# bhavyageethika/multimodal_autonomous_driving_perception_and_planning

Measured on AMD Instinct MI355X. Metric: end-to-end frames/sec (1280x720 synthetic), higher is better.
Workload: dtype f64; 1 GPU; config4: 64 stream(s)/GPU x 1-frame window per step, 1280x720, simulated detection + IoU tracker + 6-state KF + 21-candidate planner, one launch per step, up to 4 consecutive steps in flight; streams_per_gpu=64, window=1, graph=False, taggers=False, allgather_track_tables=False, fused_step=True, overlapped_steps=4, steps_per_library_call=8, parallelism=stream-sharded x1

## Files before the change

### include/avhot.h

```cpp
#ifndef AVHOT_H
#define AVHOT_H

#include <stddef.h>
#include <stdint.h>

#ifdef __cplusplus
extern "C" {
#endif

#define AV_VERSION 102

enum {
    AV_OK = 0,
    AV_EINVAL = -1,
    AV_EHIP = -2,
    AV_ENODEV = -3,
    AV_ESTATE = -4,
    AV_ENOMEM = -5
};

typedef struct av_ctx av_ctx;
typedef void* av_stream_t;

int av_version(void);
// ... 320 lines not shown
    int32_t type;
    int32_t x0, y0, x1, y1, x2, y2, x3, y3;
    int32_t p;
    uint8_t b, g, r, a;
    int32_t reserved;
} av_prim;
int av_raster_draw(av_ctx* ctx, av_stream_t stream, int n_images, int h, int w, uint8_t* img, const av_prim* prims, int prim_cap,
                   const int32_t* n_prims, const int32_t* verts, int vert_cap);
typedef struct {
    int32_t width, height;
    double pixels_per_meter;
    double x_min, x_max, y_min, y_max;
    int32_t n_candidates;
    int32_t reserved;
} av_bev_cfg;
int av_bev_prim_cap(const av_bev_cfg* cfg, int tcap, int n_points);
int av_bev_build(av_ctx* ctx, av_stream_t stream, const av_bev_cfg* cfg, int n_streams, int n_frames, int frame, int tcap,
                 int trajectory_length, const av_track_row* snap, const int32_t* snap_n, const void* tracker_state,
                 const double* vstate, const double* waypoints, const int32_t* order, av_prim* prims, int prim_cap, int32_t* n_prims);
int av_resize_into(av_ctx* ctx, av_stream_t stream, const uint8_t* src, int sh, int sw, uint8_t* dst, int dh, int dw, int dst_pitch_px,
                   int dst_x0);

int av_i420_to_bgr(av_ctx* ctx, av_stream_t stream, int n_frames, int h, int w, const uint8_t* yuv, uint8_t* bgr);

int av_synth_frames(av_ctx* ctx, av_stream_t stream, int n_streams, int h, int w, int stream0, int frame,
                    uint8_t* bgr);

int av_hot_step(av_ctx* ctx, av_stream_t stream, const av_tracker_cfg* tracker_cfg, const av_kf_cfg* kf_cfg, int n_streams, int h,
                int w, int dcap, int tcap, int32_t* frame_count, int32_t* det_n, int32_t* det_box, int32_t* det_cls,
                double* det_conf, int32_t* det_status, void* tracker_state, av_track_row* snap, int32_t* snap_n, int32_t* det2trk,
                const double* z, double* kf_state, double* vstate, double* plan_state, double* waypoints, double* cost,
                int32_t* order, void* wire, int stream0, int frame0);
int av_hot_step_fits(av_ctx* ctx, int n_streams, int dcap, int tcap, int depth);

#define AV_STEP_FLAG_INTS(n_streams) (65 * (n_streams) + 32 + 64)
int av_hot_step_seq(av_ctx* ctx, av_stream_t stream, const av_tracker_cfg* tracker_cfg, const av_kf_cfg* kf_cfg, int n_streams, int h,
                    int w, int dcap, int tcap, int32_t* frame_count, int32_t* det_n, int32_t* det_box, int32_t* det_cls,
                    double* det_conf, int32_t* det_status, void* tracker_state, av_track_row* snap, int32_t* snap_n, int32_t* det2trk,
                    const double* z, double* kf_state, double* vstate, double* plan_state, double* waypoints, double* cost,
                    int32_t* order, void* wire, int stream0, int frame0, int32_t* seq_flags, int seq, int depth);

#define AV_STEP_MAX_DEPTH 4
typedef struct av_step_set {
    int32_t *det_n, *det_box, *det_cls;
    double* det_conf;
    av_track_row* snap;
    int32_t *snap_n, *det2trk;
    const double* z;
    double *vstate, *plan_state, *waypoints, *cost;
    int32_t* order;
} av_step_set;
int av_hot_steps_seq(av_ctx* ctx, int depth, const av_stream_t* streams, const av_tracker_cfg* tracker_cfg, const av_kf_cfg* kf_cfg,
                     int n_streams, int h, int w, int dcap, int tcap, int32_t* frame_count, int32_t* det_status, void* tracker_state,
                     double* kf_state, const av_step_set* sets, const double* z_steps, void* wire_steps, int stream0, int frame0,
                     int32_t* seq_flags, int seq0, int n_steps);

#ifdef __cplusplus
}
#endif
#endif
```

### multimodal_autonomous_driving_perception_and_planning_amd/_native.py

```python
import ctypes as C
import os

_HERE = os.path.dirname(os.path.abspath(__file__))
LIB_PATH = os.path.join(_HERE, "libavhot.so")

c_i32p = C.POINTER(C.c_int32)
c_f64p = C.POINTER(C.c_double)
vp = C.c_void_p


class TrackerCfg(C.Structure):
    _fields_ = [("iou_threshold", C.c_double), ("max_age", C.c_int32), ("min_hits", C.c_int32),
                ("trajectory_length", C.c_int32)]


class KfCfg(C.Structure):
    _fields_ = [("dt", C.c_double), ("process_noise", C.c_double), ("measurement_noise", C.c_double)]


class PlannerCfg(C.Structure):
    _fields_ = [("planning_horizon", C.c_double), ("dt", C.c_double), ("num_samples", C.c_int32),
                ("reserved", C.c_int32), ("w_lateral", C.c_double), ("w_velocity", C.c_double),
                ("w_acceleration", C.c_double), ("w_curvature", C.c_double)]

# ... 84 lines not shown
    ("av_stream_sync", C.c_int, [vp]),
    ("av_stream_sync_spin", C.c_int, [vp]),
    ("av_host_alloc", C.c_int, [C.POINTER(vp), C.c_size_t]),
    ("av_host_free", C.c_int, [vp]),
    ("av_copy_h2d", C.c_int, [vp, vp, C.c_size_t, vp]),
    ("av_copy_d2h", C.c_int, [vp, vp, C.c_size_t, vp, C.c_int]),
    ("av_simdet_generate", C.c_int, [vp, vp, C.c_int, C.c_int, C.c_int, C.c_int, C.c_int, vp, vp, vp, vp, vp, vp]),
    ("av_tracker_state_bytes", C.c_size_t, [C.c_int, C.c_int]),
    ("av_tracker_reset", C.c_int, [vp, vp, C.c_int, C.c_int, C.c_int, vp]),
    ("av_tracker_update", C.c_int, [vp, vp, C.POINTER(TrackerCfg), C.c_int, C.c_int, C.c_int, vp, vp, vp, vp,
                                    C.c_int, vp, vp, vp, vp]),
    ("av_wire_table_bytes", C.c_size_t, [C.c_int]),
    ("av_pack_tracks", C.c_int, [vp, vp, C.c_int, C.c_int, C.c_int, C.c_int, C.c_int, C.c_int, C.c_int, vp, vp, vp, vp]),
    ("av_comm_unique_id", C.c_int, [vp]),
    ("av_comm_create", C.c_int, [vp, vp, C.c_int, C.c_int, C.POINTER(vp)]),
    ("av_comm_destroy", C.c_int, [vp]),
    ("av_allgather_tracks", C.c_int, [vp, vp, vp, vp, vp, C.c_size_t]),
    ("av_kf_reset", C.c_int, [vp, vp, C.c_int, vp]),
    ("av_kf_step", C.c_int, [vp, vp, C.POINTER(KfCfg), C.c_int, C.c_int, vp, vp, vp, vp, vp]),
    ("av_planner_configure", C.c_int, [vp, C.POINTER(PlannerCfg)]),
    ("av_planner_dims", C.c_int, [vp, C.POINTER(C.c_int), C.POINTER(C.c_int)]),
    ("av_planner_launch_shape", C.c_int, [C.c_int, C.c_int, C.c_int, C.c_int, c_i32p]),
    ("av_planner_plan", C.c_int, [vp, vp, C.c_int, vp, vp, C.c_int, vp, C.c_int, vp, vp, vp]),
    ("av_planner_plan_each", C.c_int, [vp, vp, C.c_int, vp, vp, vp, C.c_int, C.c_int, vp, vp, C.c_int, vp, vp, vp]),
    ("av_track_obstacles", C.c_int, [vp, vp, C.POINTER(ObstacleCfg), C.c_int, C.c_int, vp, vp, vp, C.c_int, vp, vp]),
    ("av_planner_plan_moving", C.c_int, [vp, vp, C.c_int, vp, vp, vp, C.c_int, C.c_int, vp, vp, C.c_int, vp, vp, vp]),
    ("av_track_obstacles_moving", C.c_int, [vp, vp, C.POINTER(ObstacleCfg), C.c_double, C.c_int, C.c_int, vp, vp, vp, C.c_int, vp,
                                            vp]),
    ("av_dets_to_tracker", C.c_int, [vp, vp, C.c_int, C.c_int, vp, vp, vp, vp, vp, C.c_int, C.c_int, vp, vp, vp, vp, vp]),
    ("av_lane_paths", C.c_int, [vp, vp, C.POINTER(ObstacleCfg), C.c_int, C.c_int, C.c_int, C.c_int, vp, vp, vp, vp, C.c_int,
                                C.c_int, vp, vp, vp]),
    ("av_hot_step", C.c_int, [vp, vp, C.POINTER(TrackerCfg), C.POINTER(KfCfg)] + [C.c_int] * 5 + [vp] * 17 + [vp, C.c_int, C.c_int]),
    ("av_hot_step_fits", C.c_int, [vp, C.c_int, C.c_int, C.c_int, C.c_int]),
    ("av_hot_steps_seq", C.c_int, [vp, C.c_int, vp, C.POINTER(TrackerCfg), C.POINTER(KfCfg)] + [C.c_int] * 5 + [vp] * 7 +
     [C.c_int, C.c_int, vp, C.c_int, C.c_int]),
    ("av_hot_step_seq", C.c_int, [vp, vp, C.POINTER(TrackerCfg), C.POINTER(KfCfg)] + [C.c_int] * 5 + [vp] * 17 +
     [vp, C.c_int, C.c_int, vp, C.c_int, C.c_int]),
    ("av_planner_generate", C.c_int, [vp, vp, C.c_int, vp, vp, vp, vp]),
    ("av_planner_evaluate", C.c_int, [vp, vp, C.c_int, C.c_int, vp, vp, C.c_int, vp, C.c_int, vp]),
    ("av_planner_evaluate_moving", C.c_int, [vp, vp, C.c_int, C.c_int, vp, vp, C.c_int, vp, C.c_int, vp]),
    ("av_lane_workspace_bytes", C.c_size_t, [C.c_int, C.c_int, C.c_int, C.c_int]),
    ("av_lane_workspace_init", C.c_int, [vp, vp, C.c_int, C.c_int, C.c_int, C.c_int, vp]),
    ("av_lane_workspace_view", C.c_int, [C.c_int, C.c_int, C.c_int, C.c_int, C.c_int, C.POINTER(C.c_size_t),
                                         C.POINTER(C.c_size_t)]),
    ("av_raster_draw", C.c_int, [vp, vp, C.c_int, C.c_int, C.c_int, vp, vp, C.c_int, vp, vp, C.c_int]),
    ("av_bev_prim_cap", C.c_int, [vp, C.c_int, C.c_int]),
    ("av_bev_build", C.c_int, [vp, vp, vp, C.c_int, C.c_int, C.c_int, C.c_int, C.c_int, vp, vp, vp, vp, vp, vp, vp, C.c_int, vp]),
    ("av_i420_to_bgr", C.c_int, [vp, vp, C.c_int, C.c_int, C.c_int, vp, vp]),
    ("av_resize_into", C.c_int, [vp, vp, vp, C.c_int, C.c_int, vp, C.c_int, C.c_int, C.c_int, C.c_int]),
    ("av_synth_frames", C.c_int, [vp, vp, C.c_int, C.c_int, C.c_int, C.c_int, C.c_int, vp]),
    ("av_maneuver_reset", C.c_int, [vp, vp, C.c_int, vp]),
    ("av_interaction_state_bytes", C.c_size_t, [C.c_int]),
    ("av_interaction_reset", C.c_int, [vp, vp, C.c_int, C.c_int, vp]),
    ("av_interaction_detect", C.c_int, [vp, vp, vp, C.c_int, C.c_int, C.c_int, vp, vp, vp, vp, vp, vp, vp, vp]),
    ("av_maneuver_detect", C.c_int, [vp, vp, C.c_int, C.c_int, vp, vp, vp, vp]),
    ("av_yolo_param_count", C.c_size_t, []),
    ("av_yolo_create", C.c_int, [vp, C.c_int, C.c_int, C.c_int, vp, C.c_size_t, C.POINTER(vp)]),
    ("av_yolo_create_ex", C.c_int, [vp, C.c_int, C.c_int, C.c_int, vp, C.c_size_t, C.c_int, C.POINTER(vp)]),
    ("av_yolo_destroy", C.c_int, [vp]),
    ("av_yolo_dims", C.c_int, [vp, C.POINTER(C.c_int), C.POINTER(C.c_int), C.POINTER(C.c_int)]),
    ("av_yolo_forward", C.c_int, [vp, vp, vp, C.c_float, C.c_float, C.c_int, vp, vp, vp, vp]),
    ("av_yolo_keep_logits", C.c_int, [vp, C.c_int]),
    ("av_yolo_defer_tail", C.c_int, [vp, C.c_int]),
    ("av_yolo_join_tail", C.c_int, [vp, vp]),
    ("av_yolo_tensor", C.c_int, [vp, C.c_int, C.POINTER(vp)] + [C.POINTER(C.c_int)] * 5),
    ("av_lane_detect", C.c_int, [vp, vp, C.POINTER(LaneCfg), C.c_int, C.c_int, C.c_int, vp, vp, vp, vp, vp, vp, vp,
# ... 41 lines not shown
    except OSError:
        pass


def lib():
    global _lib
    if _lib is not None:
        return _lib
    if not os.path.exists(LIB_PATH):
        raise ImportError(
            "libavhot.so is missing (%s). Build it with `python -c 'import __graft_entry__ as g; g.build()'` "
            "-- this package has no CPU fallback." % LIB_PATH)
    _preload_hip_runtime()
    L = C.CDLL(LIB_PATH)
    for name, res, args in _SIGS + _OPTIONAL_SIGS:
        fn = getattr(L, name)
        fn.restype = res
        fn.argtypes = args
    _lib = L
    return L


def register(sigs):
    global _lib
    _OPTIONAL_SIGS.extend(sigs)
    if _lib is not None:
        for name, res, args in sigs:
            fn = getattr(_lib, name)
            fn.restype = res
            fn.argtypes = args


def step_flag_ints(n_streams):
    return 65 * n_streams + 32 + 64


def step_i32(v):
    v &= 0xFFFFFFFF
    return v - (1 << 32) if v & 0x80000000 else v


class StepSet(C.Structure):
    _fields_ = [(k, C.c_void_p) for k in ("det_n", "det_box", "det_cls", "det_conf", "snap", "snap_n", "det2trk", "z", "vstate",
                                          "plan_state", "waypoints", "cost", "order")]


def check(rc):
    if rc != 0:
        raise RuntimeError("libavhot: %s (code %d)" % (lib().av_last_error_string().decode(), rc))


def ptr(t):
    if t is None:
        return None
    return C.c_void_p(t.data_ptr())


class Context:

    def __init__(self, device=0):
        L = lib()
        h = vp()
        check(L.av_ctx_create(int(device), C.byref(h)))
        self.handle = h
        self.device = int(device)
        s = vp()
        check(L.av_side_stream(h, C.byref(s)))
# ... 32 lines not shown
```

### multimodal_autonomous_driving_perception_and_planning_amd/csrc/planner.hip

```cpp
#include "common.h"

#include <cmath>



namespace {

struct PlanParams {
    int n, n_lat, C;
    double dt, H;
    double w_lat, w_vel, w_acc, w_curv;
    const double *t, *alpha, *q, *dtd, *lat;
    double atq[20];
};

static const double ATAN_Q[20] = {
    -0x1.5555555555549p-2, 0x1.99999999979b9p-3,  -0x1.24924923e22b4p-3, 0x1.c71c718e5a102p-4,
    -0x1.745d120df88fbp-4, 0x1.3b1362fc35ab5p-4,  -0x1.110deef367776p-4, 0x1.e1b3c8d50e91fp-5,
    -0x1.ae2c7119eb922p-5, 0x1.81fdd2525246ap-5,  -0x1.56daf4786fd80p-5, 0x1.2575526b2309ap-5,
    -0x1.d168e01adf666p-6, 0x1.462cc26bda000p-6,  -0x1.8055065b73333p-7, 0x1.693bd6b79999ap-8,
    -0x1.fdf4e15cccccdp-10, 0x1.f224118000000p-12, -0x1.2568700000000p-14, 0x1.2ed799999999ap-18,
};

__device__ __forceinline__ double atan2_fast(double y, double x, const double (&Q)[20]) {
// ... 125 lines not shown
        f = __builtin_amdgcn_readfirstlane(f);
        PlanLists l{nullptr, 0, nullptr, 0};
        if (ref) {
            const int pth = f / ref_stride;
            l.n_ref = path_points(pth);
            l.ref = ref + (size_t)pth * rcap * 2;
        }
        if (obs) {
            const int k = n_obs[f];
            l.n_obs = k < 0 ? 0 : (k > ocap ? ocap : k);
            l.obs = obs + (size_t)f * ocap * OS;
        }
        return l;
    }
};
using PlanEach = PlanEachT<3>;
using PlanEachMoving = PlanEachT<5>;

template <int G, int NW, class Hook = PlanNoHook, class Lists = PlanShared>
__device__ __forceinline__ void plan_block_lists(const PlanParams& p, int f0, int n_states, const double* __restrict__ state,
                                                 const Lists lists, double* __restrict__ wp, double* __restrict__ cost,
                                                 int32_t* __restrict__ order, double* sm, int state_f0 = -1, int rot = 0,
                                                 Hook after1 = Hook()) {
    const int n = p.n, C = p.C;
    const int sd = state_f0 < 0 ? 0 : state_f0 - f0;
    double* vs = sm;
    double* base = vs + (size_t)G * 3 * n * 2;
    double* trig = base + even_up(G * 3 * 3);
    double* costs = trig + G * 8;
    double* stage_all = costs + 3 * even_up(G * C);
    const int CS = even_up(G * C);

    const int tid = threadIdx.x, lane = tid & 63;
    double* stage = stage_all + (size_t)(tid >> 6) * n * 6;
    const int wid = ((tid >> 6) + NW - rot) % NW;
    constexpr int P = G * 3;
    static_assert(NW >= 2, "the heading terms take the last wave");

    auto bcast = [&](double x, int i) {
        const unsigned lo = (unsigned)__builtin_amdgcn_readlane((int)(unsigned)__double_as_longlong(x), i);
        const unsigned hi = (unsigned)__builtin_amdgcn_readlane((int)(unsigned)((unsigned long long)__double_as_longlong(x) >> 32), i);
        return __longlong_as_double((long long)(((unsigned long long)hi << 32) | lo));
    };
    auto terms = [&](double v0, double dv, int i, double& v, double& vdt, double& velt, double& acct) {
        v = blend_velocity(v0, dv, p.alpha[i]);
        vdt = v * p.dt;
        velt = velocity_term(p.w_vel, v);
        acct = 0.0;
        if (i > 0)
            acct = acceleration_term(p.w_acc, v, blend_velocity(v0, dv, p.alpha[i - 1]), p.dtd[i]);
    };
    auto cost_chains = [&](double velt, double acct, unsigned long long hasm, double* b) {
        double sv = 0.0;
#pragma unroll
        for (int i = 0; i < 64; ++i)
            if (i < n) sv = sv + bcast(velt, i);
        double run = sv, sa = 0.0;
#pragma unroll
        for (int i = 1; i < 64; ++i)
            if (i < n && ((hasm >> i) & 1ull)) {
                const double term = bcast(acct, i);
                run = run + term, sa = sa + term;
            }
        if (lane == 0) b[0] = sv, b[1] = sa, b[2] = run;
    };

    const bool fast = n <= 64 && P <= NW;
    double k_velt = 0.0, k_acct = 0.0;
    unsigned long long k_has = 0;
    bool k_live = false;
    if (fast) {
        if (wid < P) {
            const int g = wid / 3, k = wid - g * 3, f = f0 + g;
            if (f < n_states) {
                const double v0 = state[(size_t)(f + sd) * 4 + 3];
                const double dv = target_speed(k) - v0;
                double* o = vs + ((size_t)(g * 3 + k) * n) * 2;
                double v = 0.0, vdt = 0.0;
                bool has = false;
                if (lane < n) terms(v0, dv, lane, v, vdt, k_velt, k_acct), has = lane > 0 && p.dtd[lane] > 0.0;
                k_has = __ballot(has), k_live = true;
                double sacc = 0.0, my_s = 0.0;
#pragma unroll
                for (int i = 1; i < 64; ++i)
                    if (i < n) {
                        sacc = sacc + bcast(vdt, i);
                        my_s = lane == i ? sacc : my_s;
                    }
                if (lane < n) o[2 * lane] = v, o[2 * lane + 1] = my_s;
            }
        }
    } else {
        for (int pr = wid; pr < P; pr += NW) {
// ... 623 lines not shown
```

### multimodal_autonomous_driving_perception_and_planning_amd/csrc/step.hip

```cpp
#define AVHOT_DEVICE_ONLY
#include "simdet.hip"
#include "tracker.hip"
#include "kf.hip"
#include "planner.hip"
#undef AVHOT_DEVICE_ONLY

namespace {

struct StepArgs {
    int S, h, w, dcap, tcap;
    av_tracker_cfg tcfg;
    av_kf_cfg kcfg;
    PlanParams pp;
    int32_t* frame_count; const SimRow* tab; const double* cdf;
    int32_t *det_n, *det_box, *det_cls; double* det_conf; int32_t* det_status;
    unsigned char* trk_state; av_track_row* snap; int32_t* snap_n; int32_t* det2trk;
    const double* z; double *kf_state, *vstate, *plan_state;
    double *wp, *cost; int32_t* order;
    uint8_t* wire; int stream0, frame0;
    int* flags; int seq, spin, fence, stage_off;
};

constexpr int STEP_NW = 8;

__device__ __host__ inline int flag_fault(int S) { return 64 * S; }
__device__ __host__ inline int flag_base(int S) { return 64 * S + 32; }
__device__ __host__ inline int flag_stats(int S) { return 65 * S + 32; }
struct StepClock {
    unsigned long long t;
    bool on;
    unsigned long long* acc;
    __device__ void start(const StepArgs& a, int role);
    __device__ void mark(int k) {
        if (!on) return;
        const unsigned long long n = __builtin_amdgcn_s_memrealtime();
        atomicAdd(acc + k, n - t);
        t = n;
    }
};

__device__ void StepClock::start(const StepArgs& a, int role) {
    on = a.flags && (a.fence & 8) && threadIdx.x == 0;
    if (!on) return;
    acc = reinterpret_cast<unsigned long long*>(a.flags + flag_stats(a.S)) + role * 16;
    t = __builtin_amdgcn_s_memrealtime();
    atomicAdd(acc + 15, 1ull);
}

__device__ __forceinline__ bool seq_enter(const StepArgs& a, int slot, int* go) {
    if (threadIdx.x == 0) {
        int ok = 0;
        int* const counter = a.flags + 32 * slot;
        int* const fault = a.flags + flag_fault(a.S);
        const int want = a.seq, spin = a.spin;
        for (int n = 0; n <= spin; ++n) {
            if ((int)((unsigned)__hip_atomic_load(counter, __ATOMIC_RELAXED, __HIP_MEMORY_SCOPE_AGENT) - (unsigned)want) >= 0) { ok = 1; break; }
            if ((n & 255) == 255 && __hip_atomic_load(fault, __ATOMIC_RELAXED, __HIP_MEMORY_SCOPE_AGENT) != 0) break;
        }
        if (!ok) atomicOr(a.flags + flag_fault(a.S), 1);
        if (ok && (a.fence & 8) && a.seq != 0) {
            const unsigned long long tp = __hip_atomic_load(reinterpret_cast<unsigned long long*>(a.flags + 32 * slot + 2), __ATOMIC_RELAXED,
                                                            __HIP_MEMORY_SCOPE_AGENT);
            const unsigned long long now = __builtin_amdgcn_s_memrealtime();
            unsigned long long* acc = reinterpret_cast<unsigned long long*>(a.flags + flag_stats(a.S)) + (slot & 1) * 16;
            if (now > tp) atomicAdd(acc + 8, now - tp), atomicAdd(acc + 9, 1ull);
        }
        *go = ok;
    }
    __syncthreads();
    if (!*go) return false;
    if (a.fence & 1) __builtin_amdgcn_fence(__ATOMIC_ACQUIRE, "agent");
    return true;
}
__device__ __forceinline__ void seq_leave(const StepArgs& a, int slot) {
    if (a.fence & 2) __builtin_amdgcn_fence(__ATOMIC_RELEASE, "agent");
    if (a.fence & 8)
        __hip_atomic_store(reinterpret_cast<unsigned long long*>(a.flags + 32 * slot + 2), __builtin_amdgcn_s_memrealtime(), __ATOMIC_RELAXED,
                           __HIP_MEMORY_SCOPE_AGENT);
    __hip_atomic_store(a.flags + 32 * slot, (int)((unsigned)a.seq + 1u), __ATOMIC_RELAXED, __HIP_MEMORY_SCOPE_AGENT);
}
__device__ __forceinline__ void fetch_record(const void* src, void* dst_lds, int n8, int first, int end, bool coherent) {
    unsigned long long* g = const_cast<unsigned long long*>(reinterpret_cast<const unsigned long long*>(src));
    unsigned long long* l = reinterpret_cast<unsigned long long*>(dst_lds);
    if ((int)threadIdx.x < first || (int)threadIdx.x >= end) return;
    for (int i = (int)threadIdx.x - first; i < n8; i += end - first)
        l[i] = coherent ? __hip_atomic_load(g + i, __ATOMIC_RELAXED, __HIP_MEMORY_SCOPE_AGENT) : g[i];
}

template <int PW>
__global__ void __launch_bounds__(PW * 64) hot_step_kernel(StepArgs a) {
    extern __shared__ __attribute__((aligned(16))) unsigned char smem[];
    __shared__ int go, fc_stage;
    __shared__ __attribute__((aligned(16))) double kf_stage[AV_KF_STATE_DOUBLES + 2];
    __shared__ __attribute__((aligned(32))) double kf_start[4];
    __shared__ __attribute__((aligned(16))) double kf_carry[KF_CARRY_DOUBLES];
    __shared__ int kf_tail;
    __shared__ __attribute__((aligned(16))) int d_box[8 * 4];
    __shared__ __attribute__((aligned(16))) double d_conf[8], d_area[8], z_stage[4];
    __shared__ int d_cls[8], d_n[1];
    const int tid = threadIdx.x;
    const bool seq = a.flags != nullptr;
    if ((int)blockIdx.x < a.S) {
        if (PW > STEP_NW && tid >= STEP_NW * 64) return;
        const int s = blockIdx.x;
        StepClock ck;
        ck.start(a, 0);
        int fc_before = 0;
        if (tid == 0) {
            fc_before = seq ? (int)((unsigned)a.flags[flag_base(a.S) + s] + (unsigned)a.seq) : a.frame_count[s];
            fc_stage = fc_before;
            simdet_frame<true>(0, 0, 0, a.h, a.w, a.dcap, &fc_stage, a.tab, a.cdf, d_n, d_box, d_cls, d_conf,
                               a.det_status ? a.det_status + s : nullptr);
            for (int i = 0; i < a.dcap; ++i)
                d_area[i] = (double)(d_box[4 * i + 2] - d_box[4 * i]) * (double)(d_box[4 * i + 3] - d_box[4 * i + 1]);
        }
        ck.mark(0);
        if (seq && !seq_enter(a, 2 * s, &go)) return;
        ck.mark(1);
        unsigned char* stage = smem + a.stage_off;
        int fc0 = 0;
        if (seq && tid == 0) fc0 = __hip_atomic_load(a.frame_count + s, __ATOMIC_RELAXED, __HIP_MEMORY_SCOPE_AGENT);
        fetch_record(a.trk_state + (size_t)s * state_bytes(a.tcap, a.tcfg.trajectory_length), stage,
                     (HDR_INTS * 4 + a.tcap * (int)sizeof(av_track_row)) / 8, 64, STEP_NW * 64, seq);
        if (tid == 0) {
            if (seq) {
                if (fc0 != fc_before) atomicOr(a.flags + flag_fault(a.S), 2);
                __hip_atomic_store(a.frame_count + s, fc_stage, __ATOMIC_RELAXED, __HIP_MEMORY_SCOPE_AGENT);
            } else {
                a.frame_count[s] = fc_stage;
            }
        }
        if (seq) __builtin_amdgcn_s_waitcnt(0x0F70);
        __syncthreads();
        ck.mark(2);
        if (tid < a.dcap) {
            reinterpret_cast<int4*>(a.det_box)[(size_t)s * a.dcap + tid] = reinterpret_cast<const int4*>(d_box)[tid];
            a.det_cls[(size_t)s * a.dcap + tid] = d_cls[tid];
            a.det_conf[(size_t)s * a.dcap + tid] = d_conf[tid];
            if (tid == 0) a.det_n[s] = d_n[0];
        }
        tracker_body<false, 8, STEP_NW>(a.tcfg, 1, a.dcap, d_n, d_box, d_cls, d_conf, a.tcap, a.trk_state, a.snap, a.snap_n,
                                        a.det2trk, 1, s, smem, 0xFEDCBA9876543210ull, stage, seq, 0,
                                        seq ? a.flags + 32 * (2 * s) : nullptr, (int)((unsigned)a.seq + 1u), (a.fence & 8) != 0, d_area);
        ck.mark(3);
        if (a.wire) {
            __syncthreads();
            if (tid < a.tcap)
                wire_put(a.wire + (size_t)s * (AV_WIRE_HDR_BYTES + (size_t)a.tcap * AV_WIRE_ROW_BYTES), tid, a.snap_n[s], a.tcap,
                         a.snap + (size_t)s * a.tcap, a.stream0 + s, a.frame0 + fc_stage);
        }
    } else {
        const int s = blockIdx.x - a.S;
        StepClock ck;
        ck.start(a, 1);
        if (tid < 4) z_stage[tid] = a.z[(size_t)s * 4 + tid];
        if (seq && !seq_enter(a, 2 * s + 1, &go)) return;
        ck.mark(1);
        double *vs = a.vstate + (size_t)s * AV_VSTATE_DOUBLES, *ps = a.plan_state + (size_t)s * 4;
        if (tid < 64) {
            double* rec = a.kf_state + (size_t)s * AV_KF_STATE_DOUBLES;
            fetch_record(rec, kf_stage, AV_KF_STATE_DOUBLES, 0, 64, seq);
            __builtin_amdgcn_fence(__ATOMIC_RELEASE, "workgroup", "local");
            __builtin_amdgcn_wave_barrier();
            __builtin_amdgcn_fence(__ATOMIC_ACQUIRE, "workgroup", "local");
            ck.mark(2);
            const bool separable = kf_axis_chain1(a.kcfg, z_stage, kf_stage, kf_start, kf_carry, tid);
            if (tid == 0) {
                kf_tail = separable;
                if (!separable) {
                    kf_dense_stream_lds(a.kcfg, 0, 1, z_stage, nullptr, kf_stage, vs, kf_start);
                    *reinterpret_cast<double4*>(ps) = *reinterpret_cast<const double4*>(kf_start);
                }
            }
            __builtin_amdgcn_fence(__ATOMIC_RELEASE, "workgroup", "local");
            __builtin_amdgcn_wave_barrier();
            __builtin_amdgcn_fence(__ATOMIC_ACQUIRE, "workgroup", "local");
            if (tid < AV_KF_STATE_DOUBLES) {
                if (seq)
                    __hip_atomic_store(reinterpret_cast<unsigned long long*>(rec) + tid, (unsigned long long)__double_as_longlong(kf_stage[tid]),
                                       __ATOMIC_RELAXED, __HIP_MEMORY_SCOPE_AGENT);
                else
                    rec[tid] = kf_stage[tid];
            }
        }
        ck.mark(3);
        __syncthreads();
        ck.mark(4);
        constexpr int KF_ROT = 4;
        static_assert(KF_ROT + 3 < PW, "wave 0 must not be a phase-1 pair wave nor the heading wave (task wave PW - 1)");
        if (seq && tid < 64) {
            __builtin_amdgcn_s_waitcnt(0x0F70);
            if (tid == 0) seq_leave(a, 2 * s + 1);
        }
        ck.mark(5);
        const bool clocks = seq && (a.fence & 8);
        auto tail = [&](int task_wave) {
            if (task_wave != 0 || !kf_tail) return;
            const unsigned long long t0 = clocks ? __builtin_amdgcn_s_memrealtime() : 0ull;
            kf_axis_tail1(a.kcfg, kf_stage, kf_carry, vs, ps, tid & 63);
            if (clocks && (tid & 63) == 0)
                atomicAdd(reinterpret_cast<unsigned long long*>(a.flags + flag_stats(a.S)) + 16 + 7, __builtin_amdgcn_s_memrealtime() - t0);
        };
        plan_block<1, PW>(a.pp, s, a.S, kf_start, nullptr, 0, nullptr, 0, a.wp, a.cost, a.order, reinterpret_cast<double*>(smem), 0, KF_ROT,
                          tail);
        ck.mark(6);
    }
}

}

static size_t hot_step_tracker_lds(int dcap, int tcap, int& stage_off) {
    static_assert(STEP_NW == 8, "tracker_lds_bytes sizes the replica kernel's eight column waves");
    const size_t lds_t = (tracker_lds_bytes(tcap, dcap, 1, true, 0) + 15) & ~size_t(15);
    stage_off = (int)lds_t;
    return lds_t + HDR_INTS * 4 + (size_t)tcap * sizeof(av_track_row);
}

static size_t hot_step_static_lds(const void* kernel) {
    hipFuncAttributes fa{};
    return hipFuncGetAttributes(&fa, kernel) == hipSuccess ? (size_t)fa.sharedSizeBytes : (size_t)16384;
}

static int hot_step_shape(const av_ctx* ctx, int n_streams, size_t lds_t, int depth, size_t& lds_out, int& pw_out) {
    static const size_t lds_static16 = hot_step_static_lds(reinterpret_cast<const void*>(hot_step_kernel<16>));
    static const size_t lds_static8 = hot_step_static_lds(reinterpret_cast<const void*>(hot_step_kernel<8>));
    const char* pwe = getenv("AVHOT_STEP_PW");
    int pw = pwe && atoi(pwe) == 8 ? 8 : 16;
    size_t lds = 0;
    for (;;) {
        const size_t lds_p = plan_lds_doubles(1, ctx->n_points, ctx->n_cand, pw) * 8;
        lds = lds_t > lds_p ? lds_t : lds_p;
        const size_t lds_static = pw == 16 ? lds_static16 : lds_static8;
        if (lds + lds_static > 64 * 1024) {
            AV_REQUIRE(pw == 16 && !pwe, AV_EINVAL,
                       "av_hot_step: configuration needs %zu B of dynamic + %zu B of static LDS (limit 65536)", lds, lds_static);
            pw = 8;
            continue;
        }
        if (depth <= 1) break;
        int per_cu = 0;
        if (pw == 16) AV_HIP(hipOccupancyMaxActiveBlocksPerMultiprocessor(&per_cu, hot_step_kernel<16>, 16 * 64, lds));
        else AV_HIP(hipOccupancyMaxActiveBlocksPerMultiprocessor(&per_cu, hot_step_kernel<8>, 8 * 64, lds));
        if ((long long)depth * 2 * n_streams <= (long long)per_cu * ctx->n_cus) break;
        AV_REQUIRE(pw == 16 && !pwe, AV_EINVAL, "av_hot_step: %d launches of %d workgroups in flight do not fit the device (%d per CU x %d CUs)",
                   depth, 2 * n_streams, per_cu, ctx->n_cus);
        pw = 8;
    }
    lds_out = lds, pw_out = pw;
    return AV_OK;
}

static int hot_step_args(av_ctx* ctx, const av_tracker_cfg* tcfg, const av_kf_cfg* kcfg, int n_streams, int h,
                           int w, int dcap, int tcap, int32_t* frame_count, int32_t* det_n, int32_t* det_box, int32_t* det_cls,
                           double* det_conf, int32_t* det_status, void* tracker_state, av_track_row* snap, int32_t* snap_n,
                           int32_t* det2trk, const double* z, double* kf_state, double* vstate, double* plan_state,
                           double* waypoints, double* cost, int32_t* order, void* wire, int stream0, int frame0, int32_t* seq_flags,
                           int seq, StepArgs& a, size_t& lds_out, int& pw_out, int depth = 1) {
    AV_REQUIRE(ctx && tcfg && kcfg && frame_count && det_n && det_box && det_cls && det_conf && tracker_state && z && kf_state &&
                   vstate && plan_state && cost && order,
               AV_EINVAL, "av_hot_step: null argument");
    AV_REQUIRE(n_streams > 0, AV_EINVAL, "av_hot_step: n_streams must be > 0");
    AV_REQUIRE(ctx->planner_ready && ctx->d_simtab, AV_ESTATE, "av_hot_step: call av_planner_configure first");
    AV_REQUIRE((snap == nullptr) == (snap_n == nullptr), AV_EINVAL, "av_hot_step: snap and snap_n go together");
    AV_REQUIRE(!wire || snap, AV_EINVAL, "av_hot_step: the wire tables are made from the snapshot rows");
    AV_REQUIRE(tcap == 64 && dcap >= 7 && dcap <= 8 && tcfg->iou_threshold > 0.0 && tcfg->trajectory_length >= 1, AV_EINVAL,
               "av_hot_step: needs tcap 64, dcap 7..8 and iou_threshold > 0 (use the stage calls otherwise)");
    AV_REQUIRE(h > 0 && w > 121, AV_EINVAL, "av_hot_step: frame %dx%d too small", w, h);
    a = StepArgs{};
    a.S = n_streams, a.h = h, a.w = w, a.dcap = dcap, a.tcap = tcap;
    a.tcfg = *tcfg, a.kcfg = *kcfg;
    fill_params(ctx, a.pp);
    a.frame_count = frame_count, a.tab = (const SimRow*)ctx->d_simtab, a.cdf = ctx->d_cdf;
    a.det_n = det_n, a.det_box = det_box, a.det_cls = det_cls, a.det_conf = det_conf, a.det_status = det_status;
    a.trk_state = (unsigned char*)tracker_state, a.snap = snap, a.snap_n = snap_n, a.det2trk = det2trk;
    a.z = z, a.kf_state = kf_state, a.vstate = vstate, a.plan_state = plan_state;
    a.wp = waypoints, a.cost = cost, a.order = order;
    a.wire = (uint8_t*)wire, a.stream0 = stream0, a.frame0 = frame0;
    a.flags = seq_flags, a.seq = seq;
    const char* spe = seq_flags ? getenv("AVHOT_STEP_SPIN") : nullptr;
    a.spin = spe ? atoi(spe) : (1 << 22);
    const char* fe = seq_flags ? getenv("AVHOT_STEP_FENCE") : nullptr;
    a.fence = fe ? atoi(fe) : 0;
    int stage_off = 0;
    const size_t lds_t = hot_step_tracker_lds(dcap, tcap, stage_off);
    a.stage_off = stage_off;
    return hot_step_shape(ctx, n_streams, lds_t, depth, lds_out, pw_out);
}

static int hot_step_go(const StepArgs& a, size_t lds, int pw, av_stream_t stream) {
    if (pw == 16) hipLaunchKernelGGL(hot_step_kernel<16>, dim3(2 * a.S), dim3(16 * 64), lds, as_stream(stream), a);
    else hipLaunchKernelGGL(hot_step_kernel<8>, dim3(2 * a.S), dim3(8 * 64), lds, as_stream(stream), a);
    AV_LAUNCH_CHECK();
    return AV_OK;
}

static int hot_step_launch(av_ctx* ctx, av_stream_t stream, const av_tracker_cfg* tcfg, const av_kf_cfg* kcfg, int n_streams, int h,
                           int w, int dcap, int tcap, int32_t* frame_count, int32_t* det_n, int32_t* det_box, int32_t* det_cls,
                           double* det_conf, int32_t* det_status, void* tracker_state, av_track_row* snap, int32_t* snap_n,
                           int32_t* det2trk, const double* z, double* kf_state, double* vstate, double* plan_state,
                           double* waypoints, double* cost, int32_t* order, void* wire, int stream0, int frame0, int32_t* seq_flags,
                           int seq, int depth = 1) {
    StepArgs a;
    size_t lds;
    int pw;
    const int rc = hot_step_args(ctx, tcfg, kcfg, n_streams, h, w, dcap, tcap, frame_count, det_n, det_box, det_cls, det_conf, det_status,
                                 tracker_state, snap, snap_n, det2trk, z, kf_state, vstate, plan_state, waypoints, cost, order, wire, stream0,
                                 frame0, seq_flags, seq, a, lds, pw, depth);
    return rc != AV_OK ? rc : hot_step_go(a, lds, pw, stream);
}

extern "C" int av_hot_step_fits(av_ctx* ctx, int n_streams, int dcap, int tcap, int depth) {
    AV_REQUIRE(ctx && n_streams > 0 && depth >= 1, AV_EINVAL, "av_hot_step_fits: bad argument");
    AV_REQUIRE(ctx->planner_ready, AV_ESTATE, "av_hot_step_fits: call av_planner_configure first");
    AV_REQUIRE(tcap == 64 && dcap >= 7 && dcap <= 8, AV_EINVAL, "av_hot_step_fits: needs tcap 64, dcap 7..8");
    AV_HIP(hipSetDevice(ctx->device));
    int stage_off = 0;
    size_t lds = 0;
    int pw = 0;
    return hot_step_shape(ctx, n_streams, hot_step_tracker_lds(dcap, tcap, stage_off), depth, lds, pw);
}

extern "C" int av_hot_step(av_ctx* ctx, av_stream_t stream, const av_tracker_cfg* tcfg, const av_kf_cfg* kcfg, int n_streams, int h,
                           int w, int dcap, int tcap, int32_t* frame_count, int32_t* det_n, int32_t* det_box, int32_t* det_cls,
                           double* det_conf, int32_t* det_status, void* tracker_state, av_track_row* snap, int32_t* snap_n,
                           int32_t* det2trk, const double* z, double* kf_state, double* vstate, double* plan_state,
                           double* waypoints, double* cost, int32_t* order, void* wire, int stream0, int frame0) {
    return hot_step_launch(ctx, stream, tcfg, kcfg, n_streams, h, w, dcap, tcap, frame_count, det_n, det_box, det_cls, det_conf, det_status,
                           tracker_state, snap, snap_n, det2trk, z, kf_state, vstate, plan_state, waypoints, cost, order, wire, stream0,
                           frame0, nullptr, 0);
}

extern "C" int av_hot_step_seq(av_ctx* ctx, av_stream_t stream, const av_tracker_cfg* tcfg, const av_kf_cfg* kcfg, int n_streams, int h,
                               int w, int dcap, int tcap, int32_t* frame_count, int32_t* det_n, int32_t* det_box, int32_t* det_cls,
                               double* det_conf, int32_t* det_status, void* tracker_state, av_track_row* snap, int32_t* snap_n,
                               int32_t* det2trk, const double* z, double* kf_state, double* vstate, double* plan_state,
                               double* waypoints, double* cost, int32_t* order, void* wire, int stream0, int frame0,
                               int32_t* seq_flags, int seq, int depth) {
    AV_REQUIRE(seq_flags, AV_EINVAL, "av_hot_step_seq: needs the sequence flags (AV_STEP_FLAG_INTS(n_streams) int32)");
    AV_REQUIRE(depth >= 2 && depth <= AV_STEP_MAX_DEPTH, AV_EINVAL, "av_hot_step_seq: depth %d not in [2, %d]", depth, AV_STEP_MAX_DEPTH);
    return hot_step_launch(ctx, stream, tcfg, kcfg, n_streams, h, w, dcap, tcap, frame_count, det_n, det_box, det_cls, det_conf, det_status,
                           tracker_state, snap, snap_n, det2trk, z, kf_state, vstate, plan_state, waypoints, cost, order, wire, stream0,
                           frame0, seq_flags, seq, depth);
}

extern "C" int av_hot_steps_seq(av_ctx* ctx, int depth, const av_stream_t* streams, const av_tracker_cfg* tcfg, const av_kf_cfg* kcfg,
                                int n_streams, int h, int w, int dcap, int tcap, int32_t* frame_count, int32_t* det_status,
                                void* tracker_state, double* kf_state, const av_step_set* sets, const double* z_steps, void* wire_steps,
                                int stream0, int frame0, int32_t* seq_flags, int seq0, int n_steps) {
    AV_REQUIRE(seq_flags && n_steps > 0 && sets && streams, AV_EINVAL, "av_hot_steps_seq: bad argument");
    AV_REQUIRE(depth >= 2 && depth <= AV_STEP_MAX_DEPTH, AV_EINVAL, "av_hot_steps_seq: depth %d not in [2, %d]", depth, AV_STEP_MAX_DEPTH);
    for (int k = 0; k < depth; ++k)
        for (int j = 0; j < k; ++j)
// ... 24 lines not shown
```

### multimodal_autonomous_driving_perception_and_planning_amd/pipeline.py

```python
import ctypes as C

import numpy as np
import torch

from . import _native as nat


class HotLoop:
    def __init__(self, n_streams=1, window=1, h=720, w=1280, tcap=64, dcap=8, device=0,
                 tracker_kw=None, kf_kw=None, planner_kw=None, keep_waypoints=True, keep_snapshots=True,
                 ctx=None, fused_step=None, overlap=1, obstacles=None, obstacle_kw=None):
        if not torch.cuda.is_available():
            raise RuntimeError("HotLoop needs a HIP device; this package has no CPU path")
        self.S, self.W, self.h, self.w, self.tcap, self.dcap = n_streams, window, h, w, tcap, dcap
        self.dev = torch.device("cuda", device)
        self.ctx = ctx or nat.Context(device)
        self.L = nat.lib()
        tk = dict(iou_threshold=0.3, max_age=30, min_hits=3, trajectory_length=50)
        tk.update(tracker_kw or {})
        self.tcfg = nat.TrackerCfg(**tk)
        kk = dict(dt=0.033, process_noise=0.1, measurement_noise=1.0)
        kk.update(kf_kw or {})
        self.kcfg = nat.KfCfg(**kk)
        pk = dict(planning_horizon=5.0, dt=0.1, num_samples=7, w_lateral=1.0, w_velocity=0.5,
# ... 74 lines not shown
            self._seq, self._stepped = 0, False
            self._csets = None
            self.reset()
            try:
                self._enqueue_step_seq()
                self.synchronize()
            except RuntimeError as e:
                raise ValueError("overlap=%d: %s" % (self.overlap, e)) from None
        self.reset()

    def _make_ocfg(self, mode):
        ok = dict(x_center=320.0, x_scale=0.03, y_far=50.0, y_scale=0.1, radius=[1.5] * 6 + [0.0] * 10)
        ok.update(self._obstacle_kw)
        if mode == "moving_tracks":
            self.frame_rate = float(ok.pop("frame_rate", 30.0))
            if not (self.frame_rate > 0.0 and np.isfinite(self.frame_rate)):
                raise ValueError("obstacle_kw: frame_rate must be > 0 and finite")
        elif "frame_rate" in ok:
            raise ValueError('obstacle_kw: frame_rate belongs to obstacles="moving_tracks"')
        rad = [float(r) for r in ok.pop("radius")]
        if len(rad) > 16:
            raise ValueError("obstacle_kw: at most 16 per-class radii")
        return nat.ObstacleCfg(radius=(C.c_double * 16)(*(rad + [0.0] * (16 - len(rad)))), **ok)

    _PER_STEP = ("det_n", "det_box", "det_cls", "det_conf", "snap", "snap_n", "det2trk", "z", "vstate", "plan_state", "wp",
                 "cost", "order")

    @property
    def _s(self):
        return C.c_void_p(self.stream.cuda_stream)

    _i32 = staticmethod(nat.step_i32)

    def _serial_only(self, what):
        if self.overlap != 1:
            raise RuntimeError("%s is not available with overlap=2.. (only the one-launch step is ordered across the loop's streams)" % what)

    def reset(self, frame_offsets=None):
        h, L = self.ctx.handle, self.L
        if self.overlap > 1:
            for st in self._pstreams:
                st.synchronize()
        nat.check(L.av_tracker_reset(h, self._s, self.S, self.tcap, self.tcfg.trajectory_length, nat.ptr(self.trk_state)))
        nat.check(L.av_kf_reset(h, self._s, self.S, nat.ptr(self.kf_state)))
        with torch.cuda.stream(self.stream):
            if frame_offsets is None:
                self.frame_count.zero_()
            else:
                self.frame_count.copy_(torch.as_tensor(np.asarray(frame_offsets, np.int32)), non_blocking=False)
            if self.overlap > 1:
                self.seq_flags.zero_()
                self.seq_flags[64 * self.S + 32:65 * self.S + 32].copy_(self.frame_count)
        if self.overlap > 1:
            self._seq, self._stepped = 0, False
            self.__dict__.update(self._sets[0])
        self.stream.synchronize()

    def load_measurements(self, z, all_sets=False):
        if self.overlap > 1:
            zt = torch.as_tensor(np.ascontiguousarray(z, np.float64)).view(self.S, self.W, 4)
            for k in (range(self.overlap) if all_sets else (self._seq % self.overlap,)):
                with torch.cuda.stream(self._pstreams[k]):
                    self._sets[k]["z"].copy_(zt)
                self._pstreams[k].synchronize()
            self.z = self._sets[self._seq % self.overlap]["z"]
            return
# ... 709 lines not shown
```

Measured before the change: 13.30 million frames/s.

## Add 12-wave fused step variant with occupancy hint and fallback ladder

Adds a 12-wave instantiation of the fused step kernel with a waves-per-EU attribute, and the shape search now steps 16→12→8 instead of 16→8 when LDS or in-flight occupancy doesn't fit. It also reads args from the kernarg segment to keep them in scalar registers, makes the phase clock lighter (LDS timestamp, 64-bit aligned stats), makes the planner wave index uniform, and drops a redundant bound check in the scan loop. The aim is to keep more waves per workgroup when 16 won't fit with 4 steps in flight, at the cost of another kernel variant and register pressure limits.

Result: faster. 13.84 million frames/s (median of 6 runs) (+4.0%).

```diff
diff --git a/include/avhot.h b/include/avhot.h
--- a/include/avhot.h
+++ b/include/avhot.h
@@ -376,8 +376,9 @@
                 const double* z, double* kf_state, double* vstate, double* plan_state, double* waypoints, double* cost,
                 int32_t* order, void* wire, int stream0, int frame0);
 int av_hot_step_fits(av_ctx* ctx, int n_streams, int dcap, int tcap, int depth);
-
-#define AV_STEP_FLAG_INTS(n_streams) (65 * (n_streams) + 32 + 64)
+int av_hot_step_plan(av_ctx* ctx, int n_streams, int dcap, int tcap, int depth, int* waves, int* per_cu, size_t* lds_bytes);
+
+#define AV_STEP_FLAG_INTS(n_streams) (65 * (n_streams) + ((n_streams) & 1) + 32 + 64)
 int av_hot_step_seq(av_ctx* ctx, av_stream_t stream, const av_tracker_cfg* tracker_cfg, const av_kf_cfg* kf_cfg, int n_streams, int h,
                     int w, int dcap, int tcap, int32_t* frame_count, int32_t* det_n, int32_t* det_box, int32_t* det_cls,
                     double* det_conf, int32_t* det_status, void* tracker_state, av_track_row* snap, int32_t* snap_n, int32_t* det2trk,
diff --git a/multimodal_autonomous_driving_perception_and_planning_amd/_native.py b/multimodal_autonomous_driving_perception_and_planning_amd/_native.py
--- a/multimodal_autonomous_driving_perception_and_planning_amd/_native.py
+++ b/multimodal_autonomous_driving_perception_and_planning_amd/_native.py
@@ -140,6 +140,8 @@
                                 C.c_int, vp, vp, vp]),
     ("av_hot_step", C.c_int, [vp, vp, C.POINTER(TrackerCfg), C.POINTER(KfCfg)] + [C.c_int] * 5 + [vp] * 17 + [vp, C.c_int, C.c_int]),
     ("av_hot_step_fits", C.c_int, [vp, C.c_int, C.c_int, C.c_int, C.c_int]),
+    ("av_hot_step_plan", C.c_int, [vp, C.c_int, C.c_int, C.c_int, C.c_int, C.POINTER(C.c_int), C.POINTER(C.c_int),
+                                   C.POINTER(C.c_size_t)]),
     ("av_hot_steps_seq", C.c_int, [vp, C.c_int, vp, C.POINTER(TrackerCfg), C.POINTER(KfCfg)] + [C.c_int] * 5 + [vp] * 7 +
      [C.c_int, C.c_int, vp, C.c_int, C.c_int]),
     ("av_hot_step_seq", C.c_int, [vp, vp, C.POINTER(TrackerCfg), C.POINTER(KfCfg)] + [C.c_int] * 5 + [vp] * 17 +
@@ -247,7 +249,13 @@
 
 
 def step_flag_ints(n_streams):
-    return 65 * n_streams + 32 + 64
+    return 65 * n_streams + (n_streams & 1) + 32 + 64
+
+
+def step_plan(ctx_handle, n_streams, dcap, tcap, depth):
+    w, p, b = C.c_int(), C.c_int(), C.c_size_t()
+    rc = lib().av_hot_step_plan(ctx_handle, n_streams, dcap, tcap, depth, C.byref(w), C.byref(p), C.byref(b))
+    return rc, w.value, p.value, b.value
 
 
 def step_i32(v):
diff --git a/multimodal_autonomous_driving_perception_and_planning_amd/csrc/planner.hip b/multimodal_autonomous_driving_perception_and_planning_amd/csrc/planner.hip
--- a/multimodal_autonomous_driving_perception_and_planning_amd/csrc/planner.hip
+++ b/multimodal_autonomous_driving_perception_and_planning_amd/csrc/planner.hip
@@ -181,8 +181,9 @@
     const int CS = even_up(G * C);
 
     const int tid = threadIdx.x, lane = tid & 63;
-    double* stage = stage_all + (size_t)(tid >> 6) * n * 6;
-    const int wid = ((tid >> 6) + NW - rot) % NW;
+    const int wave = __builtin_amdgcn_readfirstlane(tid >> 6);
+    double* stage = stage_all + (size_t)wave * n * 6;
+    const int wid = (wave + NW - rot) % NW;
     constexpr int P = G * 3;
     static_assert(NW >= 2, "the heading terms take the last wave");
 
@@ -207,7 +208,7 @@
         double run = sv, sa = 0.0;
 #pragma unroll
         for (int i = 1; i < 64; ++i)
-            if (i < n && ((hasm >> i) & 1ull)) {
+            if ((hasm >> i) & 1ull) {
                 const double term = bcast(acct, i);
                 run = run + term, sa = sa + term;
             }
diff --git a/multimodal_autonomous_driving_perception_and_planning_amd/csrc/step.hip b/multimodal_autonomous_driving_perception_and_planning_amd/csrc/step.hip
--- a/multimodal_autonomous_driving_perception_and_planning_amd/csrc/step.hip
+++ b/multimodal_autonomous_driving_perception_and_planning_amd/csrc/step.hip
@@ -25,27 +25,34 @@
 
 __device__ __host__ inline int flag_fault(int S) { return 64 * S; }
 __device__ __host__ inline int flag_base(int S) { return 64 * S + 32; }
-__device__ __host__ inline int flag_stats(int S) { return 65 * S + 32; }
+__device__ __host__ constexpr int flag_stats(int S) { return 65 * S + (S & 1) + 32; }
+static_assert(flag_stats(1) % 2 == 0 && flag_stats(3) % 2 == 0 && flag_stats(64) % 2 == 0 && flag_stats(1) + 64 == AV_STEP_FLAG_INTS(1) &&
+                  flag_stats(3) + 64 == AV_STEP_FLAG_INTS(3) && flag_stats(64) + 64 == AV_STEP_FLAG_INTS(64),
+              "the phase clocks are the last 64 words of AV_STEP_FLAG_INTS and start at an even word");
 struct StepClock {
-    unsigned long long t;
-    bool on;
-    unsigned long long* acc;
-    __device__ void start(const StepArgs& a, int role);
-    __device__ void mark(int k) {
-        if (!on) return;
+    const StepArgs& a;
+    int role;
+    unsigned long long* t;
+    __device__ __forceinline__ bool on() const {
+        int fence = a.fence;
+        asm volatile("" : "+s"(fence));
+        return (fence & 8) && a.flags && threadIdx.x == 0;
+    }
+    __device__ __forceinline__ unsigned long long* acc() const {
+        return reinterpret_cast<unsigned long long*>(a.flags + flag_stats(a.S)) + role * 16;
+    }
+    __device__ __forceinline__ void start() {
+        if (!on()) return;
+        *t = __builtin_amdgcn_s_memrealtime();
+        atomicAdd(acc() + 15, 1ull);
+    }
+    __device__ __forceinline__ void mark(int k) {
+        if (!on()) return;
         const unsigned long long n = __builtin_amdgcn_s_memrealtime();
-        atomicAdd(acc + k, n - t);
-        t = n;
+        atomicAdd(acc() + k, n - *t);
+        *t = n;
     }
 };
-
-__device__ void StepClock::start(const StepArgs& a, int role) {
-    on = a.flags && (a.fence & 8) && threadIdx.x == 0;
-    if (!on) return;
-    acc = reinterpret_cast<unsigned long long*>(a.flags + flag_stats(a.S)) + role * 16;
-    t = __builtin_amdgcn_s_memrealtime();
-    atomicAdd(acc + 15, 1ull);
-}
 
 __device__ __forceinline__ bool seq_enter(const StepArgs& a, int slot, int* go) {
     if (threadIdx.x == 0) {
@@ -87,10 +94,17 @@
         l[i] = coherent ? __hip_atomic_load(g + i, __ATOMIC_RELAXED, __HIP_MEMORY_SCOPE_AGENT) : g[i];
 }
 
+__device__ __forceinline__ const StepArgs& role_args() {
+    auto p = __builtin_amdgcn_kernarg_segment_ptr();
+    asm volatile("" : "+s"(p));
+    return *(const StepArgs*)p;
+}
+
 template <int PW>
-__global__ void __launch_bounds__(PW * 64) hot_step_kernel(StepArgs a) {
+__device__ __forceinline__ void hot_step_body(const StepArgs& a0) {
     extern __shared__ __attribute__((aligned(16))) unsigned char smem[];
     __shared__ int go, fc_stage;
+    __shared__ unsigned long long ck_t;
     __shared__ __attribute__((aligned(16))) double kf_stage[AV_KF_STATE_DOUBLES + 2];
     __shared__ __attribute__((aligned(32))) double kf_start[4];
     __shared__ __attribute__((aligned(16))) double kf_carry[KF_CARRY_DOUBLES];
@@ -99,12 +113,13 @@
     __shared__ __attribute__((aligned(16))) double d_conf[8], d_area[8], z_stage[4];
     __shared__ int d_cls[8], d_n[1];
     const int tid = threadIdx.x;
-    const bool seq = a.flags != nullptr;
-    if ((int)blockIdx.x < a.S) {
+    const bool seq = a0.flags != nullptr;
+    if ((int)blockIdx.x < a0.S) {
+        const StepArgs& a = role_args();
         if (PW > STEP_NW && tid >= STEP_NW * 64) return;
         const int s = blockIdx.x;
-        StepClock ck;
-        ck.start(a, 0);
+        StepClock ck{a, 0, &ck_t};
+        ck.start();
         int fc_before = 0;
         if (tid == 0) {
             fc_before = seq ? (int)((unsigned)a.flags[flag_base(a.S) + s] + (unsigned)a.seq) : a.frame_count[s];
@@ -150,9 +165,10 @@
                          a.snap + (size_t)s * a.tcap, a.stream0 + s, a.frame0 + fc_stage);
         }
     } else {
+        const StepArgs& a = role_args();
         const int s = blockIdx.x - a.S;
-        StepClock ck;
-        ck.start(a, 1);
+        StepClock ck{a, 1, &ck_t};
+        ck.start();
         if (tid < 4) z_stage[tid] = a.z[(size_t)s * 4 + tid];
         if (seq && !seq_enter(a, 2 * s + 1, &go)) return;
         ck.mark(1);
@@ -207,6 +223,15 @@
     }
 }
 
+template <int PW>
+__global__ void __launch_bounds__(PW * 64) hot_step_kernel(StepArgs a) {
+    hot_step_body<PW>(a);
+}
+template <>
+__global__ void __launch_bounds__(12 * 64) __attribute__((amdgpu_waves_per_eu(6))) hot_step_kernel<12>(StepArgs a) {
+    hot_step_body<12>(a);
+}
+
 }
 
 static size_t hot_step_tracker_lds(int dcap, int tcap, int& stage_off) {
@@ -221,32 +246,38 @@
     return hipFuncGetAttributes(&fa, kernel) == hipSuccess ? (size_t)fa.sharedSizeBytes : (size_t)16384;
 }
 
-static int hot_step_shape(const av_ctx* ctx, int n_streams, size_t lds_t, int depth, size_t& lds_out, int& pw_out) {
-    static const size_t lds_static16 = hot_step_static_lds(reinterpret_cast<const void*>(hot_step_kernel<16>));
-    static const size_t lds_static8 = hot_step_static_lds(reinterpret_cast<const void*>(hot_step_kernel<8>));
+static const void* hot_step_fn(int pw) {
+    return pw == 16 ? reinterpret_cast<const void*>(hot_step_kernel<16>)
+           : pw == 12 ? reinterpret_cast<const void*>(hot_step_kernel<12>)
+                      : reinterpret_cast<const void*>(hot_step_kernel<8>);
+}
+
+static int hot_step_shape(const av_ctx* ctx, int n_streams, size_t lds_t, int depth, size_t& lds_out, int& pw_out, int* per_cu_out = nullptr) {
+    static const size_t lds_static16 = hot_step_static_lds(hot_step_fn(16));
+    static const size_t lds_static12 = hot_step_static_lds(hot_step_fn(12));
+    static const size_t lds_static8 = hot_step_static_lds(hot_step_fn(8));
     const char* pwe = getenv("AVHOT_STEP_PW");
-    int pw = pwe && atoi(pwe) == 8 ? 8 : 16;
+    const int forced = pwe ? atoi(pwe) : 0;
+    int pw = forced == 8 || forced == 12 ? forced : 16;
     size_t lds = 0;
-    for (;;) {
+    int per_cu = 0;
+    for (;; pw = pw == 16 ? 12 : 8) {
         const size_t lds_p = plan_lds_doubles(1, ctx->n_points, ctx->n_cand, pw) * 8;
         lds = lds_t > lds_p ? lds_t : lds_p;
-        const size_t lds_static = pw == 16 ? lds_static16 : lds_static8;
+        const size_t lds_static = pw == 16 ? lds_static16 : pw == 12 ? lds_static12 : lds_static8;
         if (lds + lds_static > 64 * 1024) {
-            AV_REQUIRE(pw == 16 && !pwe, AV_EINVAL,
+            AV_REQUIRE(pw > 8 && !pwe, AV_EINVAL,
                        "av_hot_step: configuration needs %zu B of dynamic + %zu B of static LDS (limit 65536)", lds, lds_static);
-            pw = 8;
             continue;
         }
         if (depth <= 1) break;
-        int per_cu = 0;
-        if (pw == 16) AV_HIP(hipOccupancyMaxActiveBlocksPerMultiprocessor(&per_cu, hot_step_kernel<16>, 16 * 64, lds));
-        else AV_HIP(hipOccupancyMaxActiveBlocksPerMultiprocessor(&per_cu, hot_step_kernel<8>, 8 * 64, lds));
+        AV_HIP(hipOccupancyMaxActiveBlocksPerMultiprocessor(&per_cu, hot_step_fn(pw), pw * 64, lds));
         if ((long long)depth * 2 * n_streams <= (long long)per_cu * ctx->n_cus) break;
-        AV_REQUIRE(pw == 16 && !pwe, AV_EINVAL, "av_hot_step: %d launches of %d workgroups in flight do not fit the device (%d per CU x %d CUs)",
+        AV_REQUIRE(pw > 8 && !pwe, AV_EINVAL, "av_hot_step: %d launches of %d workgroups in flight do not fit the device (%d per CU x %d CUs)",
                    depth, 2 * n_streams, per_cu, ctx->n_cus);
-        pw = 8;
     }
     lds_out = lds, pw_out = pw;
+    if (per_cu_out) *per_cu_out = per_cu;
     return AV_OK;
 }
 
@@ -276,6 +307,7 @@
     a.z = z, a.kf_state = kf_state, a.vstate = vstate, a.plan_state = plan_state;
     a.wp = waypoints, a.cost = cost, a.order = order;
     a.wire = (uint8_t*)wire, a.stream0 = stream0, a.frame0 = frame0;
+    AV_REQUIRE(((uintptr_t)seq_flags & 7) == 0, AV_EINVAL, "av_hot_step: the sequence flags must be 8-byte aligned (64-bit phase clocks in their last 64 words)");
     a.flags = seq_flags, a.seq = seq;
     const char* spe = seq_flags ? getenv("AVHOT_STEP_SPIN") : nullptr;
     a.spin = spe ? atoi(spe) : (1 << 22);
@@ -289,6 +321,7 @@
 
 static int hot_step_go(const StepArgs& a, size_t lds, int pw, av_stream_t stream) {
     if (pw == 16) hipLaunchKernelGGL(hot_step_kernel<16>, dim3(2 * a.S), dim3(16 * 64), lds, as_stream(stream), a);
+    else if (pw == 12) hipLaunchKernelGGL(hot_step_kernel<12>, dim3(2 * a.S), dim3(12 * 64), lds, as_stream(stream), a);
     else hipLaunchKernelGGL(hot_step_kernel<8>, dim3(2 * a.S), dim3(8 * 64), lds, as_stream(stream), a);
     AV_LAUNCH_CHECK();
     return AV_OK;
@@ -318,6 +351,21 @@
     size_t lds = 0;
     int pw = 0;
     return hot_step_shape(ctx, n_streams, hot_step_tracker_lds(dcap, tcap, stage_off), depth, lds, pw);
+}
+
+extern "C" int av_hot_step_plan(av_ctx* ctx, int n_streams, int dcap, int tcap, int depth, int* waves, int* per_cu, size_t* lds_bytes) {
+    AV_REQUIRE(ctx && n_streams > 0 && depth >= 1, AV_EINVAL, "av_hot_step_plan: bad argument");
+    AV_REQUIRE(ctx->planner_ready, AV_ESTATE, "av_hot_step_plan: call av_planner_configure first");
+    AV_REQUIRE(tcap == 64 && dcap >= 7 && dcap <= 8, AV_EINVAL, "av_hot_step_plan: needs tcap 64, dcap 7..8");
+    AV_HIP(hipSetDevice(ctx->device));
+    int stage_off = 0, pw = 0, pc = 0;
+    size_t lds = 0;
+    const int rc = hot_step_shape(ctx, n_streams, hot_step_tracker_lds(dcap, tcap, stage_off), depth, lds, pw, &pc);
+    if (rc != AV_OK) return rc;
+    if (waves) *waves = pw;
+    if (per_cu) *per_cu = pc;
+    if (lds_bytes) *lds_bytes = lds;
+    return AV_OK;
 }
 
 extern "C" int av_hot_step(av_ctx* ctx, av_stream_t stream, const av_tracker_cfg* tcfg, const av_kf_cfg* kcfg, int n_streams, int h,
diff --git a/multimodal_autonomous_driving_perception_and_planning_amd/pipeline.py b/multimodal_autonomous_driving_perception_and_planning_amd/pipeline.py
--- a/multimodal_autonomous_driving_perception_and_planning_amd/pipeline.py
+++ b/multimodal_autonomous_driving_perception_and_planning_amd/pipeline.py
@@ -130,6 +130,14 @@
 
     _i32 = staticmethod(nat.step_i32)
 
+    @property
+    def step_waves(self):
+        if not self.fused_step:
+            return None
+        rc, waves, _, _ = nat.step_plan(self.ctx.handle, self.S, self.dcap, self.tcap, self.overlap)
+        nat.check(rc)
+        return waves
+
     def _serial_only(self, what):
         if self.overlap != 1:
             raise RuntimeError("%s is not available with overlap=2.. (only the one-launch step is ordered across the loop's streams)" % what)
```
